# ZGC-SP/mpcith_kyber_kosk

Measured on AMD Instinct MI355X. Metric: kyber768_kosk_proofs_per_sec_prove_plus_verify, higher is better.
Workload: dtype u16

## Files before the change

### include/kosk_mi355x.h

```cpp
#ifndef KOSK_MI355X_H
#define KOSK_MI355X_H

#include <stddef.h>
#include <stdint.h>

#ifdef __cplusplus
extern "C" {
#endif

typedef struct kosk_ctx kosk_ctx;

typedef void (*kosk_randombytes_fn)(void *user, uint8_t *out, size_t len);

size_t kosk_pk_bytes(int kyber_k);
size_t kosk_sk_bytes(int kyber_k);
size_t kosk_proof_bytes(int kyber_k);
size_t kosk_tape_bytes(int kyber_k);
int kosk_proof_field(int kyber_k, int idx, size_t *offset, size_t *size);

#define KOSK_SEED_BYTES 32
int kosk_tape_from_seed(int kyber_k, const uint8_t seed[KOSK_SEED_BYTES], uint8_t *tape);

int kosk_create(kosk_ctx **ctx, int device, int kyber_k, int max_batch);

// ... 133 lines not shown
                        uint8_t *d_out, size_t outlen, int n);
int kosk_tape_expand_device(kosk_ctx *ctx, int n, const uint8_t *seeds, size_t seed_stride, uint8_t *d_tapes, size_t tape_stride);
int kosk_commit_hash_lanes(kosk_ctx *ctx, const uint16_t *d_rows, size_t row_stride, int n_lanes,
                           const uint8_t *d_prefix, int with_prefix, uint8_t *d_out);
int kosk_ntt256_batch(kosk_ctx *ctx, const int16_t *d_in, int16_t *d_out, int n);
int kosk_lagrange_expand(kosk_ctx *ctx, const uint16_t *d_y407, uint16_t *d_shares, int n);
int kosk_recon_secrets(kosk_ctx *ctx, const uint16_t *d_shares, uint16_t *d_secrets, int n, int two_d);
int kosk_device_synchronize(kosk_ctx *ctx);
int kosk_streams(const kosk_ctx *ctx);
int kosk_resident_proofs(kosk_ctx *ctx, void **d_proofs, size_t *stride);
int kosk_resident_digests(kosk_ctx *ctx, int round, void **d_digests, size_t *stride);
typedef void (*kosk_round_fn)(void *user, int role, int round, const void *d_digests, size_t bytes);
int kosk_set_round_hook(kosk_ctx *ctx, kosk_round_fn fn, void *user);


int kosk_keygen(int kyber_k, const uint8_t seed64[64], uint8_t *pk, uint8_t *sk,
                int16_t *A, int16_t *s, int16_t *e, int16_t *t);
int kosk_fs_alpha(int kyber_k, const uint8_t *tcomm_all, uint16_t *alpha);
int kosk_fs_opened(const uint8_t *digests_all, uint16_t *I, uint16_t *rest);
void kosk_host_sha3_256(uint8_t out[32], const uint8_t *in, size_t inlen);
void kosk_host_shake256(uint8_t *out, size_t outlen, const uint8_t *in, size_t inlen);
int kosk_host_sha3_256_multi(uint8_t *out, const uint8_t *in, size_t in_stride, size_t inlen, int count, int nthreads);
int kosk_lagrange_table(int which, uint16_t *out);

int kosk_bind_value(int kyber_k, const uint8_t *pk, const uint8_t context[32], uint8_t out[32]);
int kosk_bind_device(kosk_ctx *ctx, int n, const uint8_t *pk, const uint8_t *contexts, size_t context_stride, uint8_t *d_out);
int kosk_fs_alpha_bound(int kyber_k, const uint8_t *tcomm_all, const uint8_t bind[32], uint16_t *alpha);
int kosk_fs_opened_bound(const uint8_t *digests_all, const uint8_t bind[32], uint16_t *I, uint16_t *rest);
int kosk_fs_alpha_bound_device(kosk_ctx *ctx, const uint8_t *d_tables, size_t table_stride, int n, const uint8_t *d_bind, uint16_t *d_alpha, uint8_t *d_h1);
int kosk_fs_opened_bound_device(kosk_ctx *ctx, const uint8_t *d_tables, size_t table_stride, int n, const uint8_t *d_bind,
                                uint16_t *d_sel, uint16_t *d_rest, int sel_stride, uint8_t *d_ch);
int kosk_set_contexts(kosk_ctx *ctx, int n, const uint8_t *contexts, size_t context_stride);

#define KOSK_FORCE_MAX_LISTS 4096
int kosk_force_opened_candidates(kosk_ctx *ctx, int n, const uint16_t *cand);
int kosk_opened_tables(const uint16_t cand[150], uint16_t *sel, uint16_t *rest, int sel_stride);

int kosk_keyseed_value(int kyber_k, const uint8_t *sk, const uint8_t *context, const uint8_t *salt, uint8_t seed[32]);
int kosk_keyseed_device(kosk_ctx *ctx, int n, const uint8_t *sk, const uint8_t *contexts, size_t context_stride,
                        const uint8_t *salts, size_t salt_stride, uint8_t *d_seeds);
int kosk_stage_prover_keys_derived(kosk_ctx *ctx, int n, const uint8_t *sk, const uint8_t *salts, size_t salt_stride, uint8_t *ok);
int kosk_prove_keys_derived_batch(kosk_ctx *ctx, int n, const uint8_t *sk, const uint8_t *salts, size_t salt_stride, uint8_t *pi, uint8_t *ok);

#ifdef __cplusplus
}
#endif
// ... 2 lines not shown
```

### mpcith_kyber_kosk_amd/api.py

```python
import ctypes as C
import os

from . import build as _build

_HERE = os.path.dirname(os.path.abspath(__file__))
LIB_PATH = os.environ.get("KOSK_LIB_PATH") or os.path.join(_HERE, "libkosk_mi355x.so")


class KoskError(RuntimeError):
    pass


def _load():
    if not os.path.exists(LIB_PATH):
        _build.build()
    lib = C.CDLL(LIB_PATH)
    u8p, u16p, i16p, sz, vp = C.POINTER(C.c_uint8), C.POINTER(C.c_uint16), C.POINTER(C.c_int16), C.c_size_t, C.c_void_p
    sig = {
        "kosk_pk_bytes": (sz, [C.c_int]), "kosk_sk_bytes": (sz, [C.c_int]),
        "kosk_proof_bytes": (sz, [C.c_int]), "kosk_tape_bytes": (sz, [C.c_int]),
        "kosk_proof_field": (C.c_int, [C.c_int, C.c_int, C.POINTER(sz), C.POINTER(sz)]),
        "kosk_create": (C.c_int, [C.POINTER(vp), C.c_int, C.c_int, C.c_int]),
        "kosk_options_init": (None, [vp]),
        "kosk_create_ex": (C.c_int, [C.POINTER(vp), C.c_int, C.c_int, C.c_int, vp]),
# ... 136 lines not shown
        sig.update(wipe)
    onekey = {
        "kosk_kem_key_set": (C.c_int, [vp, vp, vp]),
        "kosk_kem_key_state": (C.c_int, [vp]),
        "kosk_kem_key_clear": (C.c_int, [vp]),
        "kosk_kem_enc_key": (C.c_int, [vp, C.c_int, vp, vp, vp]),
        "kosk_kem_dec_key": (C.c_int, [vp, C.c_int, vp, vp]),
    }
    if not (os.environ.get("KOSK_LIB_PATH") and not hasattr(lib, "kosk_kem_key_set")):
        sig.update(onekey)
    forced = {
        "kosk_force_opened_candidates": (C.c_int, [vp, C.c_int, vp]),
        "kosk_opened_tables": (C.c_int, [vp, vp, vp, C.c_int]),
    }
    if not (os.environ.get("KOSK_LIB_PATH") and not hasattr(lib, "kosk_opened_tables")):
        sig.update(forced)
    transcode = {
        "kosk_format_bytes": (sz, [C.c_int, C.c_int]),
        "kosk_transcode_batch": (C.c_int, [vp, C.c_int, C.c_int, vp, C.c_int, vp, vp]),
        "kosk_dense_check_device": (C.c_int, [vp, C.c_int, vp, sz, vp]),
    }
    if not (os.environ.get("KOSK_LIB_PATH") and not hasattr(lib, "kosk_transcode_batch")):
        sig.update(transcode)
    for name, (res, args) in sig.items():
        fn = getattr(lib, name)
        fn.restype = res
        fn.argtypes = args
    return lib


lib = _load()
EXPORTS = ["kosk_pk_bytes", "kosk_sk_bytes", "kosk_proof_bytes", "kosk_tape_bytes", "kosk_proof_field", "kosk_create",
           "kosk_destroy", "kosk_last_error", "kosk_set_randombytes", "kosk_verifiable_keygen_batch", "kosk_verify_batch",
           "kosk_verify_fail_masks", "kosk_randomness_bytes", "kosk_range_proof_bytes", "kosk_mlwe_inst_bytes",
           "kosk_prepare_randomness", "kosk_prepare_range_proof", "kosk_prove_prepared", "kosk_verify_inst", "kosk_compact_proof_bytes",
           "kosk_proof_compress", "kosk_proof_decompress", "kosk_fetch_proofs_compact", "kosk_stage_verifier_inputs_compact", "kosk_stage_prover_inputs", "kosk_prove_resident", "kosk_fetch_proofs",
           "kosk_stage_verifier_inputs", "kosk_verify_resident", "kosk_verifiable_keygen_resident", "kosk_verify_resident_pk",
           "kosk_resident_digests", "kosk_set_round_hook", "kosk_phase_seconds", "kosk_path_count", "kosk_host_threads", "kosk_sha3_256_batch_pair", "kosk_verifiable_keygen_batch_compact", "kosk_verify_batch_compact", "kosk_host_alloc", "kosk_host_free", "kosk_sha3_256_batch",
           "kosk_shake256_batch", "kosk_commit_hash_lanes", "kosk_ntt256_batch", "kosk_lagrange_expand",
           "kosk_recon_secrets", "kosk_profile_enable", "kosk_profile_read", "kosk_profile_read_units", "kosk_combine_stats", "kosk_stream_timer_start", "kosk_stream_timer_stop", "kosk_device_synchronize", "kosk_streams", "kosk_resident_proofs", "kosk_keygen", "kosk_fs_alpha",
           "kosk_fs_opened", "kosk_host_sha3_256", "kosk_host_shake256", "kosk_host_sha3_256_multi", "kosk_lagrange_table",
           "kosk_options_init", "kosk_create_ex", "kosk_sha3_256_batch_wave", "kosk_fs_alpha_device", "kosk_fs_opened_device",
           "kosk_tape_from_seed", "kosk_set_entropy", "kosk_tape_expand_device", "kosk_verifiable_keygen_seeded_batch",
           "kosk_verifiable_keygen_seeded_batch_compact", "kosk_verifiable_keygen_seeded_resident", "kosk_stage_prover_inputs_seeded",
           "kosk_ct_bytes", "kosk_kem_enc_batch", "kosk_kem_dec_batch", "kosk_kem_enc_verified",
           "kosk_witness_from_sk", "kosk_stage_prover_keys", "kosk_stage_prover_keys_seeded", "kosk_prove_keys_batch",
           "kosk_prove_keys_seeded_batch",
           "kosk_bind_value", "kosk_bind_device", "kosk_fs_alpha_bound", "kosk_fs_opened_bound", "kosk_fs_alpha_bound_device",
           "kosk_fs_opened_bound_device", "kosk_set_contexts",
           "kosk_dense_proof_bytes", "kosk_proof_dense_pack", "kosk_proof_dense_unpack", "kosk_fetch_proofs_dense",
           "kosk_stage_verifier_inputs_dense", "kosk_verifiable_keygen_batch_dense", "kosk_verifiable_keygen_seeded_batch_dense",
           "kosk_verify_batch_dense", "kosk_dense_fill_device",
           "kosk_kem_keypair_batch", "kosk_kem_check_pk", "kosk_kem_check_sk",
           "kosk_keyseed_value", "kosk_keyseed_device", "kosk_stage_prover_keys_derived", "kosk_prove_keys_derived_batch",
           "kosk_wipe_secrets", "kosk_set_wipe", "kosk_secret_scan", "kosk_wipe_device", "kosk_wipe_timing",
           "kosk_kem_key_set", "kosk_kem_key_state", "kosk_kem_key_clear", "kosk_kem_enc_key", "kosk_kem_dec_key",
           "kosk_force_opened_candidates", "kosk_opened_tables",
           "kosk_format_bytes", "kosk_transcode_batch", "kosk_dense_check_device"]
HAS_KEM = hasattr(lib, "kosk_kem_enc_batch")


class KoskOptions(C.Structure):
    _fields_ = [("size", C.c_uint32), ("streams", C.c_int32), ("combine", C.c_int32), ("combine_wait_us", C.c_int32),
                ("combine_idle_us", C.c_int32), ("combine_prewake_us", C.c_int32), ("strict_encoding", C.c_int32), ("fs_mode", C.c_int32),
# ... 816 lines not shown
```

### mpcith_kyber_kosk_amd/csrc/kosk_capi.cpp

```cpp
#include "../../include/kosk_mi355x.h"

#include <unistd.h>

#include <algorithm>
#include <condition_variable>
#include <cstdio>
#include <cstring>
#include <exception>
#include <functional>
#include <memory>
#include <mutex>
#include <string>
#include <thread>
#include <vector>

#include "kosk_combine.hpp"
#include "kosk_ctx.hpp"
#include "kosk_lanes.hpp"

using namespace kosk;

struct kosk_ctx;
struct Cohort {
    int device = 0, k = 0, per = 0;
// ... 2003 lines not shown
        sha3_256_multi(out + 32 * (size_t)lo, ptr.data() + lo, inlen, n);
    });
    return w;
    GUARD_END
}

int kosk_lagrange_table(int which, uint16_t *out)
{
    if (!out) return -1;
    return guard(static_cast<const kosk_ctx *>(nullptr), __func__, [&]() -> int {
    if (which == 0) {
        for (int x = 0; x < NPARTY - NOPEN - 1; x++) lagrange_row(out + (size_t)x * XLEN, XLEN, 0, XLEN + x);
    } else if (which == 1) {
        for (int i = 0; i < NSEC; i++) lagrange_row(out + (size_t)i * XLEN, XLEN, NSEC, i);
    } else if (which == 2) {
        for (int i = 0; i < NSEC; i++) lagrange_row(out + (size_t)i * (DEG2 + 1), DEG2 + 1, NSEC, i);
    } else {
        return -1;
    }
    return 0;
    GUARD_END
}

}
```

### mpcith_kyber_kosk_amd/csrc/kosk_ctx.cpp

```cpp
#include "kosk_ctx.hpp"

#include <atomic>

#include <chrono>
#include <cstdio>
#include <cstring>
#include <ctime>
#include <thread>

#include "kosk_math.hpp"

namespace kosk {

#define HIPCHK(x) KOSK_HIPCHK(x)

static double now_sec()
{
    return std::chrono::duration<double>(std::chrono::steady_clock::now().time_since_epoch()).count();
}

template <typename T>
static hipError_t dalloc(T **p, size_t n)
{
    return hipMalloc(reinterpret_cast<void **>(p), n * sizeof(T));
// ... 25 lines not shown
    if (ev_sync) (void)hipEventDestroy(ev_sync);
    kem_release(*this);
    transcode_release(*this);
    kem_key_release(*this);
    witness_release(*this);
    if (is_view) {
        if (h_err) (void)hipHostFree(h_err);
        if (d_compact) (void)hipFree(d_compact);
        if (d_compact_bad) (void)hipFree(d_compact_bad);
        if (h_compact) (void)hipHostFree(h_compact);
        if (h_compact_bad) (void)hipHostFree(h_compact_bad);
        if (d_dense_ws) (void)hipFree(d_dense_ws);
        if (d_dense_status) (void)hipFree(d_dense_status);
        if (pool) pool_destroy(pool);
        if (ev) (void)hipEventDestroy(ev);
        if (ev_kg) (void)hipEventDestroy(ev_kg);
        for (auto e : timer_ev)
            if (e) (void)hipEventDestroy(e);
        return;
    }
    void *dev[] = {t_expand.dfrag, t_recon_d.dfrag, t_recon_2d.dfrag, d_fresh_rows, d_gemm1_rows, d_gemm2_rows, d_off, d_fields, d_asm_groups, d_asm_elems,
                   d_rowtab, d_P, d_tape, d_seedbuf, d_dig1, d_dig2, d_proof, d_A, d_se, d_kg, d_sehat, d_t, d_alpha, d_I, d_pwT, d_coef, d_lin_rows,
                   d_gather, d_gather2, d_O, d_w, d_ell, d_sec, d_sec_u1, d_sec_u2, d_fail, d_inv, d_invlimb, d_vfields,
                   d_vrowtab, d_rows_bg, d_rows_isrc, d_rows_idst, d_rows_u, d_fact, d_invfact, d_node_of, d_isort, d_hrange, d_odig, d_bind};
    for (void *p : dev)
        if (p) (void)hipFree(p);
    void *host[] = {h_err, h_tape, h_seedbuf, h_dig, h_dig2, h_proof, h_alpha, h_I, h_fail, h_Iimg, h_kg, h_odig, h_bind};
    for (void *p : host)
        if (p) (void)hipHostFree(p);
    if (d_compact) (void)hipFree(d_compact);
    if (d_compact_bad) (void)hipFree(d_compact_bad);
    if (h_compact) (void)hipHostFree(h_compact);
    if (h_compact_bad) (void)hipHostFree(h_compact_bad);
    if (d_dense_ws) (void)hipFree(d_dense_ws);
    if (d_dense_status) (void)hipFree(d_dense_status);
    if (pool) pool_destroy(pool);
    if (ev) (void)hipEventDestroy(ev);
    if (ev_kg) (void)hipEventDestroy(ev_kg);
    for (auto e : timer_ev)
        if (e) (void)hipEventDestroy(e);
    if (stream) (void)hipStreamDestroy(stream);
}

static void pack_frag_table(const std::vector<uint16_t> &A, int M, int Kdim, int Mpad, int KS, std::vector<uint8_t> &out)
{
    const int RT = Mpad / 16;
    out.assign((size_t)KS * RT * 2048, 0);
// ... 181 lines not shown
    }
    {
        std::vector<uint16_t> A((size_t)NSEC * XLEN), A2((size_t)NSEC * (DEG2 + 1));
        for (int i = 0; i < NSEC; i++) {
            lagrange_row(&A[(size_t)i * XLEN], XLEN, NSEC, i);
            lagrange_row(&A2[(size_t)i * (DEG2 + 1)], DEG2 + 1, NSEC, i);
        }
        if (upload_table(c, c.t_recon_d, A, NSEC, XLEN)) return -1;
        if (upload_table(c, c.t_recon_2d, A2, NSEC, DEG2 + 1)) return -1;
    }

    std::vector<int16_t> fresh;
    for (int i = 0; i < M; i++) { fresh.push_back((int16_t)(rm.f + i)); fresh.push_back((int16_t)(rm.tf + i)); }
    for (int i = 0; i < K; i++)
        for (int j = 0; j < E; j++) { fresh.push_back((int16_t)(rm.seta + i * E + j)); fresh.push_back((int16_t)(rm.eeta + i * E + j)); }
    for (int i = 0; i < K; i++) { fresh.push_back((int16_t)(rm.s + i)); fresh.push_back((int16_t)(rm.e + i)); }
    for (int i = 0; i < K; i++) fresh.push_back((int16_t)(rm.nttas + i));
    for (int i = 0; i < K; i++)
        for (int j = 0; j < Z; j++) { fresh.push_back((int16_t)rm.zs(i, j)); fresh.push_back((int16_t)rm.ze(i, j)); }
    if ((int)fresh.size() != P.nfresh) { c.err = "internal: fresh row count"; return -1; }
    if (upload_vec(c, &c.d_fresh_rows, fresh)) return -1;
    if (upload_vec(c, &c.d_gemm1_rows, fresh)) return -1;
    c.n_gemm1 = (int)fresh.size();
    std::vector<int16_t> g2;
    for (int i = 0; i < K; i++) { g2.push_back((int16_t)(rm.nttsr + i)); g2.push_back((int16_t)(rm.ntter + i)); g2.push_back((int16_t)(rm.nttasr + i)); }
    if (upload_vec(c, &c.d_gemm2_rows, g2)) return -1;
    c.n_gemm2 = (int)g2.size();

    {
        std::vector<int16_t> lr(256, 0);
        for (int j = 0; j < P.J; j++) {
            lr[j] = (int16_t)(j < NCHK ? rm.beta(j) : rm.r + (j - NCHK));
            lr[128 + j] = (int16_t)(j < NCHK ? rm.gamma(j) : rm.nttr + (j - NCHK));
        }
        if (upload_vec(c, &c.d_lin_rows, lr)) return -1;
    }

    std::vector<int32_t> off;
    auto push_rows = [&](int row0, int n) { int b = (int)off.size(); for (int i = 0; i < n; i++) off.push_back((row0 + i) * RS); return b; };
    c.off_ntt1_src = push_rows(rm.f, M);
    push_rows(rm.s, K);
    c.off_ntt1_dst = push_rows(rm.tf, M);
    push_rows(rm.shat, K);
    c.n_ntt1 = M + K;
    c.off_sr_er = push_rows(rm.sr, 2 * K);
    c.off_nttsr_er = push_rows(rm.nttsr, 2 * K);
    if (rm.er != rm.sr + K || rm.ntter != rm.nttsr + K) { c.err = "internal: row map adjacency"; return -1; }
    if (upload_vec(c, &c.d_off, off)) return -1;
// ... 944 lines not shown
```

### mpcith_kyber_kosk_amd/csrc/kosk_ctx.hpp

```cpp
#pragma once
#include <hip/hip_runtime.h>

#include <string>
#include <functional>
#include <vector>

#include "kosk_device.hpp"
#include "kosk_host.hpp"
#include "kosk_params.hpp"

#define KOSK_HIPCHK(x)                                                      \
    do {                                                                    \
        hipError_t e_ = (x);                                                \
        if (e_ != hipSuccess) {                                             \
            (void)hipGetLastError();                                        \
            c.err = std::string(#x) + ": " + hipGetErrorString(e_);         \
            return -1;                                                      \
        }                                                                   \
    } while (0)

namespace kosk {

typedef void (*randombytes_fn)(void *user, uint8_t *out, size_t len);
typedef void (*round_fn)(void *user, int role, int round, const void *d_digests, size_t bytes);
// ... 163 lines not shown
    int16_t *d_sehat = nullptr;
    int resident_pk_n = 0;
    size_t pk_stride = 0, sb_stride = 0;
    unsigned long pk_epoch = 0;
    int keys_from_pk_n = 0;
    void note_pk_written(int n) { resident_pk_n = n; keys_from_pk_n = n; pk_epoch++; }
    void note_pk_decoded(int n) { if (n > keys_from_pk_n) keys_from_pk_n = n; }
    void note_keys_from_inst() { keys_from_pk_n = 0; pk_epoch++; }
    uint8_t *h_seeds = nullptr, *h_pk = nullptr, *h_sb = nullptr;
    uint16_t *d_t = nullptr;
    uint16_t *d_alpha = nullptr, *d_I = nullptr, *d_rest = nullptr;
    int32_t *d_pwT = nullptr;
    uint8_t *d_coef = nullptr;
    int16_t *d_lin_rows = nullptr;
    bool verify_ready = false;
    uint16_t *d_O = nullptr;
    size_t o_stride = 0;
    uint16_t *d_inv = nullptr;
    FieldDesc *d_vfields = nullptr;
    int16_t *d_vrowtab = nullptr;
    int n_vfields = 0;
    FieldPlan vplan{}, pplan{};
    int16_t *d_rows_bg = nullptr;
    int16_t *d_rows_isrc = nullptr, *d_rows_idst = nullptr;
    int16_t *d_rows_u = nullptr;
    int n_interp_d = 0, n_interp_2d = 0;
    uint16_t *d_w = nullptr, *d_ell = nullptr, *d_fact = nullptr, *d_invfact = nullptr;
    int16_t *d_node_of = nullptr;
    uint16_t *d_isort = nullptr, *d_hrange = nullptr;
    uint8_t *d_gather = nullptr, *d_gather2 = nullptr;
    uint16_t *d_invlimb = nullptr;
    uint16_t *d_sec = nullptr, *d_sec_u1 = nullptr, *d_sec_u2 = nullptr;
    uint32_t *d_fail = nullptr;
    uint16_t *h_Iimg = nullptr;
    uint8_t *d_odig = nullptr, *h_odig = nullptr;
    const uint8_t *host_img = nullptr;
    size_t host_img_stride = 0;
    hipEvent_t ev = nullptr;
    std::vector<uint16_t> v_I2, v_rest2;
    std::function<void()> near_end_hook;
    bool kg_on_host_pending = false;
    hipEvent_t ev_kg = nullptr;
    bool wait_nap = true;
    enum { WAIT_SITES = 8 };
    enum { WAIT_HIST = 8 };
    enum { WAIT_SIZES = 2 };
    struct WaitHist {
// ... 210 lines not shown
```

### mpcith_kyber_kosk_amd/csrc/kosk_device.hpp

```cpp
#pragma once
#include <hip/hip_runtime.h>

#include "kosk_math.hpp"
#include "kosk_params.hpp"

namespace kosk {

struct XofGuard {
    uint32_t *err = nullptr;
    int max_blocks = 32;
};
enum : uint32_t { DEVERR_XOF_BLOCKS = 1u };


struct HashArgs {
    const uint16_t *rows;
    size_t group_stride;
    int row_stride;
    int col_off;
    int lanes_per_group;
    const uint8_t *prefix;
    uint8_t *out;
    int out_lanes_per_group;
};
// ... 140 lines not shown
    const uint16_t *opened, *rest;
    int sel_stride;
    uint32_t *fail;
    int strict;
};

KOSK_HD inline uint32_t ref_add_u16(uint32_t a, uint32_t b) { const int32_t s = (int32_t)a + (int32_t)b; return (uint32_t)(s < Q ? s : s - Q) & 0xFFFFu; }
KOSK_HD inline uint32_t ref_sub_u16(uint32_t a, uint32_t b) { return (uint32_t)(a < b ? (int32_t)a + Q - (int32_t)b : (int32_t)a - (int32_t)b) & 0xFFFFu; }
KOSK_HD inline uint32_t gf_fold(uint32_t x) { return x >= (uint32_t)Q ? x % (uint32_t)Q : x; }

struct InterpArgs {
    const uint16_t *rest;
    const uint16_t *isort;
    const uint16_t *hrange;
    int sel_stride;
    const uint16_t *inv, *fact, *invfact;
    const uint16_t *invlimb;
    uint16_t *w;
    uint16_t *ell;
    int16_t *node_of;
};

hipError_t launch_opened_setup(const uint8_t *proof, size_t image_stride, size_t off_I, uint16_t *I, uint16_t *rest, uint16_t *isort,
                               uint16_t *hrange, size_t sel_stride, uint32_t *fail, int nproofs, hipStream_t st);
hipError_t launch_disassemble(const VerifyArgs &v, const FieldDesc *fields, const FieldPlan &plan, const int16_t *rowtab,
                              const uint8_t *proof, size_t image_stride, size_t off_tcomm, size_t off_comm,
                              uint8_t *dig1, uint8_t *dig2, const GateOffsets &go, int nproofs, hipStream_t st);
struct OpenedHashArgs {
    const uint8_t *proof;
    size_t image_stride;
    uint32_t off_s, off_e, off_f, off_nttf, off_zs, off_ze;
    const uint16_t *P;
    size_t proof_stride;
    const uint16_t *O;
    size_t o_stride;
    RowMap rm;
    const uint16_t *opened;
    int sel_stride;
    const uint8_t *prefix;
    uint8_t *out;
    uint8_t *out_compact;
};
hipError_t launch_opened_hash(const OpenedHashArgs &a, int K, bool view, int nproofs, hipStream_t st);
hipError_t launch_check_batch(const VerifyArgs &v, const uint16_t *t_pk, const uint16_t *u1, const uint16_t *u2, int nu, int nproofs,
                              hipStream_t st);
size_t interp_y_bytes(int set);
int interp_table_len();
// ... 119 lines not shown
```

### mpcith_kyber_kosk_amd/csrc/kosk_params.hpp

```cpp
#pragma once
#include <cstddef>
#include <cstdint>

#if defined(__HIPCC__)
#define KOSK_HD __host__ __device__
#else
#define KOSK_HD
#endif

namespace kosk {

constexpr int Q = 3329;
constexpr int NSEC = 256;
constexpr int NPARTY = 1454;
constexpr int NOPEN = 150;
constexpr int NREST = NPARTY - NOPEN;
constexpr int NCHK = 70;
constexpr int DEG = 406;
constexpr int DEG2 = 812;
constexpr int NPTS = NSEC + NPARTY;
constexpr int RS = 1728;
constexpr int XLEN = DEG + 1;
constexpr int EXP_OFF = 384;
constexpr int EXP_M = RS - EXP_OFF;
// ... 69 lines not shown
{
    RowMap r{};
    const int K = p.K, M = p.M, E = p.E, Z = p.Z;
    r.K = K; r.M = M; r.E = E; r.Z = Z;
    int n = 0;
    auto take = [&](int cnt) { int b = n; n += cnt; return b; };
    r.s = take(K); r.e = take(K); r.f = take(M); r.tf = take(M);
    r.beta0 = take(K); r.gamma0 = take(K); r.sr = take(K); r.er = take(K);
    r.gate = take(4 * Z * K);
    r.RV = n;
    r.beta1 = take(NCHK - K); r.gamma1 = take(NCHK - K);
    r.r = take(2 * K); r.nttr = take(2 * K);
    r.seta = take(K * E); r.eeta = take(K * E);
    r.nttsr = take(K); r.ntter = take(K); r.nttasr = take(K); r.nttas = take(K);
    r.ntts = take(K); r.ntte = take(K); r.nttar = take(K); r.t = take(K);
    r.ssub = take(K * E); r.esub = take(K * E);
    r.shat = take(K);
    r.sr_in = take(K); r.er_in = take(K); r.t_in = take(K);
    r.seta_in = take(K * E); r.eeta_in = take(K * E);
    r.nrows = n;
    return r;
}

}
```

### mpcith_kyber_kosk_amd/csrc/kosk_verify.cpp

```cpp
#include <atomic>
#include <cstring>
#include <functional>
#include <mutex>
#include <utility>
#include <vector>

#include "kosk_ctx.hpp"

#include <chrono>
#include "kosk_math.hpp"

namespace kosk {

static double now_sec()
{
    return std::chrono::duration<double>(std::chrono::steady_clock::now().time_since_epoch()).count();
}

#define HIPCHK(x) KOSK_HIPCHK(x)

template <typename T>
static hipError_t dalloc(T **p, size_t n) { return hipMalloc(reinterpret_cast<void **>(p), (n ? n : 1) * sizeof(T)); }
template <typename T>
static int upload_vec(Ctx &c, T **d, const std::vector<T> &v)
// ... 51 lines not shown
    add(F_GAMMA, 1, NCHK, [&](int e) { return rm.gamma(e); }, DEG + 1, 1);
    add(F_S, 0, K, [&](int e) { return rm.s + e; });
    add(F_E, 0, K, [&](int e) { return rm.e + e; });
    add(F_T, 1, K, [&](int e) { return rm.t_in + e; }, DEG + 1);
    add(F_NTTS, 0, K, [&](int e) { return rm.ntts + e; });
    add(F_NTTE, 0, K, [&](int e) { return rm.ntte + e; });
    add(F_NTTAR, 0, K, [&](int e) { return rm.nttar + e; });
    add(F_NTTAS, 0, K, [&](int e) { return rm.nttas + e; });
    add(F_SR, 1, K, [&](int e) { return rm.sr_in + e; }, 0, 0, FB_SR_ER_SHARES);
    add(F_ER, 1, K, [&](int e) { return rm.er_in + e; }, 0, 0, FB_SR_ER_SHARES);
    add(F_SETA, 1, K * E, [&](int e) { return rm.seta_in + e; }, DEG + 1);
    add(F_EETA, 1, K * E, [&](int e) { return rm.eeta_in + e; }, DEG + 1);
    add(F_SSUB, 0, K * E, [&](int e) { return rm.ssub + e; });
    add(F_ESUB, 0, K * E, [&](int e) { return rm.esub + e; });
    add(F_ZS, 0, K * Z, [&](int e) { return rm.zs(e / Z, e % Z); });
    add(F_ZE, 0, K * Z, [&](int e) { return rm.ze(e / Z, e % Z); });
    add(F_US, 1, K * Z, [&](int e) { return rm.us(e / Z, e % Z); }, DEG2 + 1);
    add(F_UE, 1, K * Z, [&](int e) { return rm.ue(e / Z, e % Z); }, DEG2 + 1);
    c.n_vfields = (int)vf.size();
    c.vplan = make_field_plan(vf.data(), c.n_vfields);
    if (upload_vec(c, &c.d_vfields, vf)) return -1;
    if (upload_vec(c, &c.d_vrowtab, rt)) return -1;

    std::vector<int16_t> bg, isrc, idst, urows;
    for (int j = 0; j < NCHK; j++) bg.push_back((int16_t)rm.beta(j));
    for (int j = 0; j < NCHK; j++) bg.push_back((int16_t)rm.gamma(j));
    auto pair = [&](int src0, int dst0, int n) { for (int i = 0; i < n; i++) { isrc.push_back((int16_t)(src0 + i)); idst.push_back((int16_t)(dst0 + i)); } };
    pair(rm.sr_in, rm.sr, K);
    pair(rm.er_in, rm.er, K);
    pair(rm.t_in, rm.t, K);
    pair(rm.seta_in, rm.seta, K * E);
    pair(rm.eeta_in, rm.eeta, K * E);
    for (int i = 0; i < K; i++) for (int k = 0; k < Z; k++) urows.push_back((int16_t)rm.us(i, k));
    for (int i = 0; i < K; i++) for (int k = 0; k < Z; k++) urows.push_back((int16_t)rm.ue(i, k));
    c.n_interp_d = (int)isrc.size();
    c.n_interp_2d = (int)urows.size();
    if (upload_vec(c, &c.d_rows_bg, bg) || upload_vec(c, &c.d_rows_isrc, isrc) || upload_vec(c, &c.d_rows_idst, idst) ||
        upload_vec(c, &c.d_rows_u, urows))
        return -1;

    c.o_stride = (size_t)rm.nrows * OS;
    auto dev = [&](auto **p, size_t per) -> hipError_t {
        const hipError_t e = dalloc(p, B * per);
        if (e == hipSuccess) { c.reg_pp(p, per * sizeof(**p)); c.reg_buf("verifier workspace", p, per * sizeof(**p), Ctx::INV_PER_PROOF, Ctx::INVG_VERIFY); }
        return e;
    };
    HIPCHK(dev(&c.d_O, c.o_stride));
    HIPCHK(hipMemsetAsync(c.d_O, 0, B * c.o_stride * sizeof(uint16_t), c.stream));
    HIPCHK(dev(&c.d_w, (size_t)2 * 832));
    HIPCHK(dev(&c.d_ell, 416));
    HIPCHK(dev(&c.d_node_of, 416));
    HIPCHK(dev(&c.d_isort, (size_t)c.sel_stride));
    HIPCHK(dev(&c.d_hrange, 4));
    HIPCHK(dev(&c.d_gather, interp_y_bytes(0)));
    HIPCHK(dev(&c.d_gather2, interp_y_bytes(1)));
    HIPCHK(dev(&c.d_sec, (size_t)2 * NCHK * 256));
    HIPCHK(dev(&c.d_sec_u1, (size_t)c.n_interp_2d * 256));
    HIPCHK(dev(&c.d_sec_u2, (size_t)c.n_interp_2d * 256));
    HIPCHK(hipHostMalloc(reinterpret_cast<void **>(&c.h_Iimg), B * 2 * NOPEN, hipHostMallocDefault));
    c.reg_pp(&c.h_Iimg, (size_t)2 * NOPEN);
// ... 102 lines not shown
    oh.proof = c.d_proof;
    oh.image_stride = c.image_stride;
    oh.off_s = (uint32_t)P.off[F_S]; oh.off_e = (uint32_t)P.off[F_E]; oh.off_f = (uint32_t)P.off[F_F];
    oh.off_nttf = (uint32_t)P.off[F_NTTF]; oh.off_zs = (uint32_t)P.off[F_ZS]; oh.off_ze = (uint32_t)P.off[F_ZE];
    oh.P = c.d_P;
    oh.proof_stride = c.proof_stride;
    oh.O = c.d_O;
    oh.o_stride = c.o_stride;
    oh.rm = rm;
    oh.opened = c.d_I;
    oh.sel_stride = c.sel_stride;
    oh.prefix = nullptr;
    oh.out = c.d_dig1;
    const bool split_tables = !c.fs_device && himg != nullptr;
    oh.out_compact = split_tables ? c.d_odig : nullptr;
    const size_t dig_bytes = split_tables ? (size_t)n * NOPEN * 32 : (size_t)n * NPARTY * 32;
    auto table_prep = [&](int r) {
        return std::function<void(int)>([&c, himg, himg_stride, r](int b) {
            const uint8_t *unopened = himg + (size_t)b * himg_stride + c.P.off[r ? F_COMM : F_TCOMM];
            assemble_digest_table(c.h_dig + (size_t)b * NPARTY * 32, c.h_Iimg + (size_t)b * NOPEN, unopened, c.h_odig + (size_t)b * NOPEN * 32);
        });
    };
    if (run_segment(c, Ctx::SEG_V1, n, [&]() -> int {
    HIPCHK(launch_opened_setup(c.d_proof, c.image_stride, P.off[F_I], c.d_I, c.d_rest, c.d_isort, c.d_hrange, c.sel_stride, c.d_fail, n, st));
    if (!c.fs_device) HIPCHK(copy_small(c, c.h_Iimg, 2 * NOPEN, c.d_proof + P.off[F_I], c.image_stride, 2 * NOPEN, n, hipMemcpyDeviceToHost, st));


    const GateOffsets go{(uint32_t)P.off[F_SSUB], (uint32_t)P.off[F_ESUB], (uint32_t)P.off[F_ZS], (uint32_t)P.off[F_ZE]};
    HIPCHK(launch_disassemble(va, c.d_vfields, c.vplan, c.d_vrowtab, c.d_proof, c.image_stride, P.off[F_TCOMM],
                              P.off[F_COMM], c.d_dig1, c.d_dig2, go, n, st));
    c.prof_begin(PR_V_HASH_TCOMM, n);
    HIPCHK(launch_opened_hash(oh, K, false, n, st));
    c.prof_end(PR_V_HASH_TCOMM);
    if (c.fs_device) return 0;
    if (split_tables) HIPCHK(hipMemcpyAsync(c.h_odig, c.d_odig, dig_bytes, hipMemcpyDeviceToHost, st));
    else HIPCHK(copy_round_table(c, c.h_dig, c.d_dig1, n));
    return 0;
    }, c.fs_device ? nullptr : split_tables ? c.h_odig : c.h_dig)) return -1;
    if (issue_bind_values(c, n)) return -1;
    HIPCHK(hipEventRecord(c.ev, st));
    if (c.fs_device) {
        FsArgs fa{};
        fa.in = c.d_dig1; fa.in_stride = (size_t)NPARTY * 32; fa.len = NPARTY * 32;
        fa.alpha = c.d_alpha; fa.alpha_stride = 80; fa.J = P.J;
        fa.bind = bound ? c.d_bind : nullptr;
        c.prof_begin(PR_V_FS_ALPHA, n);
        HIPCHK(launch_fs_chain(fa, FS_ALPHA, n, st));
        c.prof_end(PR_V_FS_ALPHA);
        c.path_n[PATH_FS_DEVICE]++;
// ... 1 lines not shown
    t1 = now_sec(); c.phase_sec[PH_V1_ISSUE] = t1 - t0; t0 = t1;

    if (run_segment(c, Ctx::SEG_V1B, n, [&]() -> int {
    if (pk_mode) HIPCHK(launch_decode_pk(c.d_pk, c.pk_stride, c.d_t, c.d_A, c.key_stride, K, n, st, c.xof_guard()));
    InterpArgs ia{};
    ia.rest = c.d_rest;
    ia.isort = c.d_isort;
    ia.hrange = c.d_hrange;
    ia.sel_stride = c.sel_stride;
    ia.inv = c.d_inv;
    ia.invlimb = c.d_invlimb;
    ia.fact = c.d_fact;
    ia.invfact = c.d_invfact;
    ia.w = c.d_w;
    ia.ell = c.d_ell;
    ia.node_of = c.d_node_of;
    c.prof_begin(PR_V_INTERP_BUILD, n);
    HIPCHK(launch_interp_setup(ia, n, st));
    c.prof_end(PR_V_INTERP_BUILD);
    HIPCHK(launch_gather_frags(c.d_P, c.proof_stride, c.d_rows_isrc, c.n_interp_d, c.d_gather, c.d_rows_u, c.n_interp_2d, c.d_gather2,
                               c.d_rest, c.sel_stride, c.d_w, n, st));
    {
        c.prof_begin(PR_V_GEMM_INTERP, n);
        HIPCHK(launch_interp_apply(ia, c.d_P, c.proof_stride, c.d_rows_isrc, c.d_rows_idst, c.n_interp_d, c.d_gather, c.n_interp_2d,
                                   c.d_gather2, c.d_sec_u1, n, st));
        c.prof_end(PR_V_GEMM_INTERP);
        const GemmSrc gs3{c.d_P, c.proof_stride, c.d_rows_u, RS, NSEC};
        const GemmDst gd3{c.d_sec_u2, (size_t)c.n_interp_2d * 256, nullptr, 256, 0};
        if (gemm_modq(c, c.t_recon_2d, gs3, gd3, c.n_interp_2d, n)) return -1;
        const GemmSrc xs{c.d_P, c.proof_stride, c.d_rows_idst, RS, 0};
        const GemmDst xd{c.d_P, c.proof_stride, c.d_rows_idst, RS, EXP_OFF};
        c.prof_begin(PR_V_GEMM_EXPAND, n);
        if (gemm_modq(c, c.t_expand, xs, xd, c.n_interp_d, n)) return -1;
        c.prof_end(PR_V_GEMM_EXPAND);
    }
    HIPCHK(launch_check_batch(va, c.d_t, c.d_sec_u1, c.d_sec_u2, c.n_interp_2d, n, st));
    NttArgs na{};
    na.in = reinterpret_cast<const int16_t *>(c.d_P);
    na.in_gstride = c.proof_stride;
    na.src_off = c.d_off + c.off_sr_er;
    na.npg = 2 * K;
    na.npoly = 2 * K * n;
    na.out = reinterpret_cast<int16_t *>(c.d_P);
    na.out_gstride = c.proof_stride;
    na.dst_off = c.d_off + c.off_nttsr_er;
    na.out_canonical = 1;
    HIPCHK(launch_relation_ntt(na, c.d_A, c.key_stride, c.d_P, c.proof_stride, rm, n, st));
    {
        const GemmSrc xs{c.d_P, c.proof_stride, c.d_gemm2_rows, RS, 0};
        const GemmDst xd{c.d_P, c.proof_stride, c.d_gemm2_rows, RS, EXP_OFF};
        if (gemm_modq(c, c.t_expand, xs, xd, c.n_gemm2, n)) return -1;
    }
    return 0;
    })) return -1;

    auto any_hook = [&]() {
        bool h = c.round_hook != nullptr;
        for (const VerifySeg *sg = segs; sg; sg = sg->next) h |= sg->hook != nullptr;
        return h;
    };
    const bool hooks = c.fs_device && any_hook();
    if (!c.fs_device || hooks) HIPCHK(wait_event(c, c.ev, 3, n));
    t1 = now_sec(); c.phase_sec[PH_V1_WAIT] = t1 - t0; t0 = t1;
    auto fire_hooks = [&](int rnd, const uint8_t *d_table) {
        bool seg_hooks = false;
        for (const VerifySeg *s = segs; s; s = s->next) seg_hooks |= s->hook != nullptr;
        if (!seg_hooks) {
            if (c.round_hook) c.round_hook(c.round_user, 1, rnd, d_table, (size_t)n * NPARTY * 32);
            return;
        }
        int first = 0;
        for (const VerifySeg *s = segs; s; s = s->next) {
            if (s->hook) s->hook(s->hook_user, 1, rnd, d_table + (size_t)first * NPARTY * 32, (size_t)s->count * NPARTY * 32);
            first += s->count;
        }
// ... 125 lines not shown
```

### mpcith_kyber_kosk_amd/csrc/kosk_verify_kernels.hip

```cpp
#include <hip/hip_runtime.h>

#include <utility>

#include "kosk_device.hpp"
#include "kosk_keccak_dev.hpp"
#include "kosk_keccak_split_dev.hpp"
#include "kosk_math.hpp"

#include <cstdlib>
#include "kosk_cauchy_dev.hpp"
#include "kosk_wave_sync_dev.hpp"

namespace kosk {

constexpr int DIS_TILE = 64 * 80;

__global__ __launch_bounds__(64) void k_disassemble_fields(VerifyArgs v, const FieldDesc *__restrict__ fields, FieldPlan plan,
                                                          const int16_t *__restrict__ rowtab,
                                                          const uint8_t *__restrict__ proof, size_t image_stride, uint32_t off_tcomm,
                                                          uint32_t off_comm, uint8_t *__restrict__ dig1, uint8_t *__restrict__ dig2,
                                                          GateOffsets go)
{
    {
        const int nfb = plan.nrest * NWIN + plan.nopen * ((NOPEN + 63) / 64) + (NREST * 4 + 63) / 64;
// ... 442 lines not shown
    for (int m = 0; m < MAXE; m++) {
        const int mm = i * E + min(m, E - 1);
        p_seta[m] = at(rm.seta + mm); p_eeta[m] = at(rm.eeta + mm);
        o_ssub[m] = op(rm.ssub + mm); o_esub[m] = op(rm.esub + mm);
    }
    uint32_t bits = 0;
    if (o_ntts != ref_sub_u16(p_nttsr, o_nttr_s)) bits |= 1u << FB_NTT_S_E;
    if (o_ntte != ref_sub_u16(p_ntter, o_nttr_e)) bits |= 1u << FB_NTT_S_E;
    if (p_nttasr != ref_add_u16(o_nttas, o_nttar)) bits |= 1u << FB_A_SR;
    if (p_t != ref_add_u16(o_nttas, o_ntte)) bits |= 1u << FB_T_RELATION;
#pragma unroll
    for (int m = 0; m < MAXE; m++) {
        if (m < E && o_ssub[m] != ref_sub_u16(o_s, p_seta[m])) bits |= 1u << FB_SUB_ETA;
        if (m < E && o_esub[m] != ref_sub_u16(o_e, p_eeta[m])) bits |= 1u << FB_SUB_ETA;
    }
    if (bits) atomicOr(&v.fail[b], bits);
}



__global__ __launch_bounds__(256) void k_opened_setup(const uint8_t *__restrict__ proof, size_t image_stride, uint32_t off_I,
                                                     uint16_t *__restrict__ I, uint16_t *__restrict__ rest,
                                                     uint16_t *__restrict__ isort, uint16_t *__restrict__ hrange,
                                                     size_t sel_stride, uint32_t *__restrict__ fail)
{
    __shared__ uint32_t cnt[NPARTY];
    __shared__ int bad, wave_used[4], node[3];
    const int t = threadIdx.x, b = blockIdx.x;
    for (int p = t; p < NPARTY; p += 256) cnt[p] = 0;
    if (t == 0) bad = 0;
    __syncthreads();
    uint32_t v = t;
    if (t < NOPEN) {
        v = reinterpret_cast<const uint16_t *>(proof + (size_t)b * image_stride + off_I)[t];
        if (v >= NPARTY || atomicAdd(&cnt[v], 1u) != 0) atomicOr(&bad, 1);
    }
    __syncthreads();
    const bool malformed = bad != 0;
    if (malformed) {
        __syncthreads();
        for (int p = t; p < NPARTY; p += 256) cnt[p] = p < NOPEN;
        v = t;
        __syncthreads();
    }
    if (t < NOPEN) I[(size_t)b * sel_stride + t] = (uint16_t)v;
    int u[6], mine = 0;
#pragma unroll
    for (int k = 0; k < 6; k++) {
        const int p = 6 * t + k;
        u[k] = p < NPARTY && cnt[p] != 0;
        mine += u[k];
    }
    int incl = mine;
#pragma unroll
    for (int d = 1; d < 64; d <<= 1) {
        const int o = __shfl_up(incl, d, 64);
        if ((t & 63) >= d) incl += o;
    }
// ... 86 lines not shown
    }
}

hipError_t launch_check_batch(const VerifyArgs &v, const uint16_t *t_pk, const uint16_t *u1, const uint16_t *u2, int nu, int nproofs,
                              hipStream_t st)
{
    hipLaunchKernelGGL(k_check_batch, dim3((NREST + 255) / 256 + 1 + 2 * nu, nproofs), dim3(256), 0, st, v, t_pk, u1, u2, nu);
    return hipGetLastError();
}
size_t interp_y_bytes(int set) { return set ? IA_Y2_BYTES : IA_Y1_BYTES; }
int interp_table_len() { return IA_TAB + 2; }
int interp_table_off() { return IA_OFF; }
hipError_t launch_gather_frags(const uint16_t *P, size_t proof_stride, const int16_t *rows1, int nrows1, uint8_t *out1,
                               const int16_t *rows2, int nrows2, uint8_t *out2, const uint16_t *rest, int sel_stride,
                               const uint16_t *w, int nproofs, hipStream_t st)
{
    if (nrows1 > 16 * IA_NT1 || nrows2 > 16 * IA_NT2) return hipErrorInvalidValue;
    const int threads = IA_NT1 * 16 * IA_KS1 * 4 + IA_NT2 * 16 * IA_KS2 * 4;
    hipLaunchKernelGGL(k_gather_frags, dim3((threads + 255) / 256, nproofs), dim3(256), 0, st, P, proof_stride, rows1, nrows1, out1, rows2,
                       nrows2, out2, rest, sel_stride, w);
    return hipGetLastError();
}
hipError_t launch_opened_setup(const uint8_t *proof, size_t image_stride, size_t off_I, uint16_t *I, uint16_t *rest, uint16_t *isort,
                               uint16_t *hrange, size_t sel_stride, uint32_t *fail, int nproofs, hipStream_t st)
{
    hipLaunchKernelGGL(k_opened_setup, dim3(nproofs), dim3(256), 0, st, proof, image_stride, (uint32_t)off_I, I, rest, isort, hrange, sel_stride, fail);
    return hipGetLastError();
}
hipError_t launch_disassemble(const VerifyArgs &v, const FieldDesc *fields, const FieldPlan &plan, const int16_t *rowtab,
                              const uint8_t *proof, size_t image_stride, size_t off_tcomm, size_t off_comm,
                              uint8_t *dig1, uint8_t *dig2, const GateOffsets &go, int nproofs, hipStream_t st)
{
    hipLaunchKernelGGL(k_disassemble_fields, dim3(plan.nrest * NWIN + plan.nopen * ((NOPEN + 63) / 64) + (NREST * 4 + 63) / 64 + (NOPEN + 63) / 64, nproofs), dim3(64), 0,
                       st, v, fields, plan, rowtab, proof, image_stride, (uint32_t)off_tcomm, (uint32_t)off_comm, dig1, dig2, go);
    return hipGetLastError();
}
hipError_t launch_interp_setup(const InterpArgs &a, int nproofs, hipStream_t st)
{
    hipLaunchKernelGGL(k_interp_setup, dim3(8 * nproofs), dim3(256), 0, st, a, nproofs);
    return hipGetLastError();
}
hipError_t launch_interp_apply(const InterpArgs &a, uint16_t *P, size_t proof_stride, const int16_t *src_rows, const int16_t *dst_rows,
                               int n1, const uint8_t *y1, int n2, const uint8_t *y2, uint16_t *out2, int nproofs, hipStream_t st)
{
    if (n1 > 16 * IA_NT1 || n2 > 16 * IA_NT2 || n1 < 1 || n2 < 1) return hipErrorInvalidValue;
    InterpApplyArgs g{};
    g.ia = a;
    g.P = P;
    g.proof_stride = proof_stride;
// ... 18 lines not shown
```

Baseline: 187,600.

## Merge verifier expansion GEMMs and write opened list to host from kernel

The two separate expansion GEMMs (interpolated rows, then resharing rows after the relation NTT) are merged into one GEMM over a combined row list that runs after the NTT. The check kernel moves after it. The opened-index list is now written straight to mapped host memory by the opened-setup kernel instead of a separate strided copy. The aim is fewer launches and copies in the verify path. The risks are a later start for the check and reliance on the host buffer being device-writable.

```diff
diff --git a/include/kosk_mi355x.h b/include/kosk_mi355x.h
--- a/include/kosk_mi355x.h
+++ b/include/kosk_mi355x.h
@@ -179,6 +179,7 @@
 void kosk_host_shake256(uint8_t *out, size_t outlen, const uint8_t *in, size_t inlen);
 int kosk_host_sha3_256_multi(uint8_t *out, const uint8_t *in, size_t in_stride, size_t inlen, int count, int nthreads);
 int kosk_lagrange_table(int which, uint16_t *out);
+int kosk_verifier_rows(int kyber_k, int which, int16_t *out, int cap);
 
 int kosk_bind_value(int kyber_k, const uint8_t *pk, const uint8_t context[32], uint8_t out[32]);
 int kosk_bind_device(kosk_ctx *ctx, int n, const uint8_t *pk, const uint8_t *contexts, size_t context_stride, uint8_t *d_out);
diff --git a/mpcith_kyber_kosk_amd/api.py b/mpcith_kyber_kosk_amd/api.py
--- a/mpcith_kyber_kosk_amd/api.py
+++ b/mpcith_kyber_kosk_amd/api.py
@@ -182,6 +182,8 @@
     }
     if not (os.environ.get("KOSK_LIB_PATH") and not hasattr(lib, "kosk_transcode_batch")):
         sig.update(transcode)
+    if not (os.environ.get("KOSK_LIB_PATH") and not hasattr(lib, "kosk_verifier_rows")):
+        sig["kosk_verifier_rows"] = (C.c_int, [C.c_int, C.c_int, vp, C.c_int])
     for name, (res, args) in sig.items():
         fn = getattr(lib, name)
         fn.restype = res
@@ -199,7 +201,7 @@
            "kosk_resident_digests", "kosk_set_round_hook", "kosk_phase_seconds", "kosk_path_count", "kosk_host_threads", "kosk_sha3_256_batch_pair", "kosk_verifiable_keygen_batch_compact", "kosk_verify_batch_compact", "kosk_host_alloc", "kosk_host_free", "kosk_sha3_256_batch",
            "kosk_shake256_batch", "kosk_commit_hash_lanes", "kosk_ntt256_batch", "kosk_lagrange_expand",
            "kosk_recon_secrets", "kosk_profile_enable", "kosk_profile_read", "kosk_profile_read_units", "kosk_combine_stats", "kosk_stream_timer_start", "kosk_stream_timer_stop", "kosk_device_synchronize", "kosk_streams", "kosk_resident_proofs", "kosk_keygen", "kosk_fs_alpha",
-           "kosk_fs_opened", "kosk_host_sha3_256", "kosk_host_shake256", "kosk_host_sha3_256_multi", "kosk_lagrange_table",
+           "kosk_fs_opened", "kosk_host_sha3_256", "kosk_host_shake256", "kosk_host_sha3_256_multi", "kosk_lagrange_table", "kosk_verifier_rows",
            "kosk_options_init", "kosk_create_ex", "kosk_sha3_256_batch_wave", "kosk_fs_alpha_device", "kosk_fs_opened_device",
            "kosk_tape_from_seed", "kosk_set_entropy", "kosk_tape_expand_device", "kosk_verifiable_keygen_seeded_batch",
            "kosk_verifiable_keygen_seeded_batch_compact", "kosk_verifiable_keygen_seeded_resident", "kosk_stage_prover_inputs_seeded",
diff --git a/mpcith_kyber_kosk_amd/csrc/kosk_capi.cpp b/mpcith_kyber_kosk_amd/csrc/kosk_capi.cpp
--- a/mpcith_kyber_kosk_amd/csrc/kosk_capi.cpp
+++ b/mpcith_kyber_kosk_amd/csrc/kosk_capi.cpp
@@ -2049,4 +2049,23 @@
     GUARD_END
 }
 
-}
+int kosk_verifier_rows(int kyber_k, int which, int16_t *out, int cap)
+{
+    Params P;
+    if (!out || !make_params(kyber_k, P)) return -1;
+    return guard(static_cast<const kosk_ctx *>(nullptr), __func__, [&]() -> int {
+    const RowMap rm = make_rowmap(P);
+    int16_t rows[MAX_EXPAND_ROWS];
+    int n;
+    if (which == 0) n = verifier_expand_rows(rm, rows);
+    else if (which == 1) n = verifier_interp_rows(rm, nullptr, rows);
+    else if (which == 2) n = resharing_rows(rm, rows);
+    else if (which == 3) n = verifier_interp_rows(rm, rows, nullptr);
+    else return -1;
+    if (n > cap) return -1;
+    memcpy(out, rows, sizeof(int16_t) * (size_t)n);
+    return n;
+    GUARD_END
+}
+
+}
diff --git a/mpcith_kyber_kosk_amd/csrc/kosk_ctx.cpp b/mpcith_kyber_kosk_amd/csrc/kosk_ctx.cpp
--- a/mpcith_kyber_kosk_amd/csrc/kosk_ctx.cpp
+++ b/mpcith_kyber_kosk_amd/csrc/kosk_ctx.cpp
@@ -71,7 +71,7 @@
     void *dev[] = {t_expand.dfrag, t_recon_d.dfrag, t_recon_2d.dfrag, d_fresh_rows, d_gemm1_rows, d_gemm2_rows, d_off, d_fields, d_asm_groups, d_asm_elems,
                    d_rowtab, d_P, d_tape, d_seedbuf, d_dig1, d_dig2, d_proof, d_A, d_se, d_kg, d_sehat, d_t, d_alpha, d_I, d_pwT, d_coef, d_lin_rows,
                    d_gather, d_gather2, d_O, d_w, d_ell, d_sec, d_sec_u1, d_sec_u2, d_fail, d_inv, d_invlimb, d_vfields,
-                   d_vrowtab, d_rows_bg, d_rows_isrc, d_rows_idst, d_rows_u, d_fact, d_invfact, d_node_of, d_isort, d_hrange, d_odig, d_bind};
+                   d_vrowtab, d_rows_bg, d_rows_isrc, d_rows_expand, d_rows_u, d_fact, d_invfact, d_node_of, d_isort, d_hrange, d_odig, d_bind};
     for (void *p : dev)
         if (p) (void)hipFree(p);
     void *host[] = {h_err, h_tape, h_seedbuf, h_dig, h_dig2, h_proof, h_alpha, h_I, h_fail, h_Iimg, h_kg, h_odig, h_bind};
@@ -299,8 +299,8 @@
     if (upload_vec(c, &c.d_fresh_rows, fresh)) return -1;
     if (upload_vec(c, &c.d_gemm1_rows, fresh)) return -1;
     c.n_gemm1 = (int)fresh.size();
-    std::vector<int16_t> g2;
-    for (int i = 0; i < K; i++) { g2.push_back((int16_t)(rm.nttsr + i)); g2.push_back((int16_t)(rm.ntter + i)); g2.push_back((int16_t)(rm.nttasr + i)); }
+    std::vector<int16_t> g2(MAX_EXPAND_ROWS);
+    g2.resize((size_t)resharing_rows(rm, g2.data()));
     if (upload_vec(c, &c.d_gemm2_rows, g2)) return -1;
     c.n_gemm2 = (int)g2.size();
 
diff --git a/mpcith_kyber_kosk_amd/csrc/kosk_ctx.hpp b/mpcith_kyber_kosk_amd/csrc/kosk_ctx.hpp
--- a/mpcith_kyber_kosk_amd/csrc/kosk_ctx.hpp
+++ b/mpcith_kyber_kosk_amd/csrc/kosk_ctx.hpp
@@ -209,7 +209,9 @@
     int n_vfields = 0;
     FieldPlan vplan{}, pplan{};
     int16_t *d_rows_bg = nullptr;
-    int16_t *d_rows_isrc = nullptr, *d_rows_idst = nullptr;
+    int16_t *d_rows_isrc = nullptr;
+    int16_t *d_rows_expand = nullptr;
+    int n_expand = 0;
     int16_t *d_rows_u = nullptr;
     int n_interp_d = 0, n_interp_2d = 0;
     uint16_t *d_w = nullptr, *d_ell = nullptr, *d_fact = nullptr, *d_invfact = nullptr;
diff --git a/mpcith_kyber_kosk_amd/csrc/kosk_device.hpp b/mpcith_kyber_kosk_amd/csrc/kosk_device.hpp
--- a/mpcith_kyber_kosk_amd/csrc/kosk_device.hpp
+++ b/mpcith_kyber_kosk_amd/csrc/kosk_device.hpp
@@ -186,7 +186,8 @@
 };
 
 hipError_t launch_opened_setup(const uint8_t *proof, size_t image_stride, size_t off_I, uint16_t *I, uint16_t *rest, uint16_t *isort,
-                               uint16_t *hrange, size_t sel_stride, uint32_t *fail, int nproofs, hipStream_t st);
+                               uint16_t *hrange, size_t sel_stride, uint32_t *fail, uint16_t *h_list, size_t h_stride, int nproofs,
+                               hipStream_t st);
 hipError_t launch_disassemble(const VerifyArgs &v, const FieldDesc *fields, const FieldPlan &plan, const int16_t *rowtab,
                               const uint8_t *proof, size_t image_stride, size_t off_tcomm, size_t off_comm,
                               uint8_t *dig1, uint8_t *dig2, const GateOffsets &go, int nproofs, hipStream_t st);
diff --git a/mpcith_kyber_kosk_amd/csrc/kosk_params.hpp b/mpcith_kyber_kosk_amd/csrc/kosk_params.hpp
--- a/mpcith_kyber_kosk_amd/csrc/kosk_params.hpp
+++ b/mpcith_kyber_kosk_amd/csrc/kosk_params.hpp
@@ -115,4 +115,37 @@
     return r;
 }
 
+constexpr int MAX_EXPAND_ROWS = (3 + 2 * 7) * MAXK + 3 * MAXK;
+inline int verifier_interp_rows(const RowMap &rm, int16_t *src, int16_t *dst)
+{
+    int n = 0;
+    auto pair = [&](int src0, int dst0, int cnt) {
+        for (int i = 0; i < cnt; i++, n++) {
+            if (src) src[n] = (int16_t)(src0 + i);
+            if (dst) dst[n] = (int16_t)(dst0 + i);
+        }
+    };
+    pair(rm.sr_in, rm.sr, rm.K);
+    pair(rm.er_in, rm.er, rm.K);
+    pair(rm.t_in, rm.t, rm.K);
+    pair(rm.seta_in, rm.seta, rm.K * rm.E);
+    pair(rm.eeta_in, rm.eeta, rm.K * rm.E);
+    return n;
 }
+inline int resharing_rows(const RowMap &rm, int16_t *out)
+{
+    int n = 0;
+    for (int i = 0; i < rm.K; i++) {
+        out[n++] = (int16_t)(rm.nttsr + i);
+        out[n++] = (int16_t)(rm.ntter + i);
+        out[n++] = (int16_t)(rm.nttasr + i);
+    }
+    return n;
+}
+inline int verifier_expand_rows(const RowMap &rm, int16_t *out)
+{
+    const int n = verifier_interp_rows(rm, nullptr, out);
+    return n + resharing_rows(rm, out + n);
+}
+
+}
diff --git a/mpcith_kyber_kosk_amd/csrc/kosk_verify.cpp b/mpcith_kyber_kosk_amd/csrc/kosk_verify.cpp
--- a/mpcith_kyber_kosk_amd/csrc/kosk_verify.cpp
+++ b/mpcith_kyber_kosk_amd/csrc/kosk_verify.cpp
@@ -97,20 +97,18 @@
     if (upload_vec(c, &c.d_vfields, vf)) return -1;
     if (upload_vec(c, &c.d_vrowtab, rt)) return -1;
 
-    std::vector<int16_t> bg, isrc, idst, urows;
+    std::vector<int16_t> bg, isrc(MAX_EXPAND_ROWS), xrows(MAX_EXPAND_ROWS), urows;
     for (int j = 0; j < NCHK; j++) bg.push_back((int16_t)rm.beta(j));
     for (int j = 0; j < NCHK; j++) bg.push_back((int16_t)rm.gamma(j));
-    auto pair = [&](int src0, int dst0, int n) { for (int i = 0; i < n; i++) { isrc.push_back((int16_t)(src0 + i)); idst.push_back((int16_t)(dst0 + i)); } };
-    pair(rm.sr_in, rm.sr, K);
-    pair(rm.er_in, rm.er, K);
-    pair(rm.t_in, rm.t, K);
-    pair(rm.seta_in, rm.seta, K * E);
-    pair(rm.eeta_in, rm.eeta, K * E);
+    isrc.resize((size_t)verifier_interp_rows(rm, isrc.data(), nullptr));
+    xrows.resize((size_t)verifier_expand_rows(rm, xrows.data()));
     for (int i = 0; i < K; i++) for (int k = 0; k < Z; k++) urows.push_back((int16_t)rm.us(i, k));
     for (int i = 0; i < K; i++) for (int k = 0; k < Z; k++) urows.push_back((int16_t)rm.ue(i, k));
     c.n_interp_d = (int)isrc.size();
+    c.n_expand = (int)xrows.size();
     c.n_interp_2d = (int)urows.size();
-    if (upload_vec(c, &c.d_rows_bg, bg) || upload_vec(c, &c.d_rows_isrc, isrc) || upload_vec(c, &c.d_rows_idst, idst) ||
+    if (c.n_expand != c.n_interp_d + c.n_gemm2) { c.err = "internal: expansion row list"; return -1; }
+    if (upload_vec(c, &c.d_rows_bg, bg) || upload_vec(c, &c.d_rows_isrc, isrc) || upload_vec(c, &c.d_rows_expand, xrows) ||
         upload_vec(c, &c.d_rows_u, urows))
         return -1;
 
@@ -259,9 +257,8 @@
         });
     };
     if (run_segment(c, Ctx::SEG_V1, n, [&]() -> int {
-    HIPCHK(launch_opened_setup(c.d_proof, c.image_stride, P.off[F_I], c.d_I, c.d_rest, c.d_isort, c.d_hrange, c.sel_stride, c.d_fail, n, st));
-    if (!c.fs_device) HIPCHK(copy_small(c, c.h_Iimg, 2 * NOPEN, c.d_proof + P.off[F_I], c.image_stride, 2 * NOPEN, n, hipMemcpyDeviceToHost, st));
-
+    HIPCHK(launch_opened_setup(c.d_proof, c.image_stride, P.off[F_I], c.d_I, c.d_rest, c.d_isort, c.d_hrange, c.sel_stride, c.d_fail,
+                               c.fs_device ? nullptr : c.h_Iimg, NOPEN, n, st));
 
     const GateOffsets go{(uint32_t)P.off[F_SSUB], (uint32_t)P.off[F_ESUB], (uint32_t)P.off[F_ZS], (uint32_t)P.off[F_ZE]};
     HIPCHK(launch_disassemble(va, c.d_vfields, c.vplan, c.d_vrowtab, c.d_proof, c.image_stride, P.off[F_TCOMM],
@@ -309,19 +306,13 @@
                                c.d_rest, c.sel_stride, c.d_w, n, st));
     {
         c.prof_begin(PR_V_GEMM_INTERP, n);
-        HIPCHK(launch_interp_apply(ia, c.d_P, c.proof_stride, c.d_rows_isrc, c.d_rows_idst, c.n_interp_d, c.d_gather, c.n_interp_2d,
+        HIPCHK(launch_interp_apply(ia, c.d_P, c.proof_stride, c.d_rows_isrc, c.d_rows_expand, c.n_interp_d, c.d_gather, c.n_interp_2d,
                                    c.d_gather2, c.d_sec_u1, n, st));
         c.prof_end(PR_V_GEMM_INTERP);
         const GemmSrc gs3{c.d_P, c.proof_stride, c.d_rows_u, RS, NSEC};
         const GemmDst gd3{c.d_sec_u2, (size_t)c.n_interp_2d * 256, nullptr, 256, 0};
         if (gemm_modq(c, c.t_recon_2d, gs3, gd3, c.n_interp_2d, n)) return -1;
-        const GemmSrc xs{c.d_P, c.proof_stride, c.d_rows_idst, RS, 0};
-        const GemmDst xd{c.d_P, c.proof_stride, c.d_rows_idst, RS, EXP_OFF};
-        c.prof_begin(PR_V_GEMM_EXPAND, n);
-        if (gemm_modq(c, c.t_expand, xs, xd, c.n_interp_d, n)) return -1;
-        c.prof_end(PR_V_GEMM_EXPAND);
-    }
-    HIPCHK(launch_check_batch(va, c.d_t, c.d_sec_u1, c.d_sec_u2, c.n_interp_2d, n, st));
+    }
     NttArgs na{};
     na.in = reinterpret_cast<const int16_t *>(c.d_P);
     na.in_gstride = c.proof_stride;
@@ -334,10 +325,13 @@
     na.out_canonical = 1;
     HIPCHK(launch_relation_ntt(na, c.d_A, c.key_stride, c.d_P, c.proof_stride, rm, n, st));
     {
-        const GemmSrc xs{c.d_P, c.proof_stride, c.d_gemm2_rows, RS, 0};
-        const GemmDst xd{c.d_P, c.proof_stride, c.d_gemm2_rows, RS, EXP_OFF};
-        if (gemm_modq(c, c.t_expand, xs, xd, c.n_gemm2, n)) return -1;
-    }
+        const GemmSrc xs{c.d_P, c.proof_stride, c.d_rows_expand, RS, 0};
+        const GemmDst xd{c.d_P, c.proof_stride, c.d_rows_expand, RS, EXP_OFF};
+        c.prof_begin(PR_V_GEMM_EXPAND, n);
+        if (gemm_modq(c, c.t_expand, xs, xd, c.n_expand, n)) return -1;
+        c.prof_end(PR_V_GEMM_EXPAND);
+    }
+    HIPCHK(launch_check_batch(va, c.d_t, c.d_sec_u1, c.d_sec_u2, c.n_interp_2d, n, st));
     return 0;
     })) return -1;
 
diff --git a/mpcith_kyber_kosk_amd/csrc/kosk_verify_kernels.hip b/mpcith_kyber_kosk_amd/csrc/kosk_verify_kernels.hip
--- a/mpcith_kyber_kosk_amd/csrc/kosk_verify_kernels.hip
+++ b/mpcith_kyber_kosk_amd/csrc/kosk_verify_kernels.hip
@@ -488,8 +488,10 @@
 __global__ __launch_bounds__(256) void k_opened_setup(const uint8_t *__restrict__ proof, size_t image_stride, uint32_t off_I,
                                                      uint16_t *__restrict__ I, uint16_t *__restrict__ rest,
                                                      uint16_t *__restrict__ isort, uint16_t *__restrict__ hrange,
-                                                     size_t sel_stride, uint32_t *__restrict__ fail)
-{
+                                                     size_t sel_stride, uint32_t *__restrict__ fail,
+                                                     uint16_t *__restrict__ h_list, size_t h_stride)
+{
+    static_assert(NOPEN % 2 == 0, "the list is stored to the host two entries at a time");
     __shared__ uint32_t cnt[NPARTY];
     __shared__ int bad, wave_used[4], node[3];
     const int t = threadIdx.x, b = blockIdx.x;
@@ -500,6 +502,10 @@
     if (t < NOPEN) {
         v = reinterpret_cast<const uint16_t *>(proof + (size_t)b * image_stride + off_I)[t];
         if (v >= NPARTY || atomicAdd(&cnt[v], 1u) != 0) atomicOr(&bad, 1);
+    }
+    if (h_list) {
+        const uint32_t up = (uint32_t)__shfl_down((int)v, 1, 64);
+        if (t < NOPEN && !(t & 1)) reinterpret_cast<uint32_t *>(h_list + (size_t)b * h_stride)[t >> 1] = v | (up << 16);
     }
     __syncthreads();
     const bool malformed = bad != 0;
@@ -632,9 +638,12 @@
     return hipGetLastError();
 }
 hipError_t launch_opened_setup(const uint8_t *proof, size_t image_stride, size_t off_I, uint16_t *I, uint16_t *rest, uint16_t *isort,
-                               uint16_t *hrange, size_t sel_stride, uint32_t *fail, int nproofs, hipStream_t st)
-{
-    hipLaunchKernelGGL(k_opened_setup, dim3(nproofs), dim3(256), 0, st, proof, image_stride, (uint32_t)off_I, I, rest, isort, hrange, sel_stride, fail);
+                               uint16_t *hrange, size_t sel_stride, uint32_t *fail, uint16_t *h_list, size_t h_stride, int nproofs,
+                               hipStream_t st)
+{
+    if (h_list && ((h_stride & 1) || (reinterpret_cast<uintptr_t>(h_list) & 3))) return hipErrorInvalidValue;
+    hipLaunchKernelGGL(k_opened_setup, dim3(nproofs), dim3(256), 0, st, proof, image_stride, (uint32_t)off_I, I, rest, isort, hrange, sel_stride, fail,
+                       h_list, h_stride);
     return hipGetLastError();
 }
 hipError_t launch_disassemble(const VerifyArgs &v, const FieldDesc *fields, const FieldPlan &plan, const int16_t *rowtab,
```

Result: slower. 181,700 (-3.2%).
